# NikolausDemmel/rootba

Hardware: NVIDIA H100
Metric: ms/LM-iter (linearize+QR+PCG) on BAL at 1/2/4/8 H100 vs CPU ref (lower is better)
Workload: dtype f32

## Files before the change

rootba_b200/csrc/assembled.cuh:

```cuda
#pragma once

#include "kernels.cuh"

namespace rba {

struct AsmTerm {
  long long base;
  int ij, meta;
};

template <class S>
__global__ void __launch_bounds__(256) k_rcs_terms(const S* __restrict__ panel, const AsmTerm* __restrict__ terms, long long w0,
                                                   long long w1, int damping, S* __restrict__ stage) {
  using V2 = typename ST<S>::V2;
  const int lane = threadIdx.x & 31;
  const int g = lane / 9, p = lane - 9 * g;
  if (lane >= 27) return;
  const long long warps = (long long)gridDim.x * (blockDim.x >> 5);
  for (long long w = w0 + 3 * (blockIdx.x * (long long)(blockDim.x >> 5) + (threadIdx.x >> 5)) + g; w < w1; w += 3 * warps) {
    const AsmTerm at = terms[w];
    const int n = at.meta & 0x7fff, lg = (at.meta >> 15) & 7, KP = at.meta >> 18, G = 1 << lg;
    const int ia = at.ij & 0xffff, ib = at.ij >> 16;
    const int ca = 9 * ia + p, pa = ca >> 1;
    const int off_a = 2 * ((pa >> lg) * 32 + (pa & (G - 1))) + (ca & 1);
    const int cb0 = 9 * ib, pb0 = cb0 >> 1;
    const bool odd = cb0 & 1;
    int off_b[5];
#pragma unroll
    for (int k = 0; k < 5; ++k) off_b[k] = ((pb0 + k) >> lg) * 32 + ((pb0 + k) & (G - 1));
    const size_t rstride = (size_t)KP * 64;
    const S* __restrict__ lmp = panel + at.base;
    const int r0 = damping ? 2 * n - 3 : 0, r1 = damping ? 2 * n : 2 * n - 3;
    S acc[9];
#pragma unroll
    for (int q = 0; q < 9; ++q) acc[q] = 0;
#pragma unroll 3
    for (int r = r0; r < r1; ++r) {
      const S* row = lmp + (size_t)r * rstride;
      const V2* row2 = reinterpret_cast<const V2*>(row);
      const S va = __ldg(row + off_a);
      V2 b[5];
#pragma unroll
      for (int k = 0; k < 5; ++k) b[k] = __ldg(row2 + off_b[k]);
      const S el[10] = {b[0].x, b[0].y, b[1].x, b[1].y, b[2].x, b[2].y, b[3].x, b[3].y, b[4].x, b[4].y};
#pragma unroll
      for (int q = 0; q < 9; ++q) acc[q] = fma(va, odd ? el[q + 1] : el[q], acc[q]);
    }
    S* o = stage + 81 * (size_t)(w - w0) + 9 * p;
#pragma unroll
    for (int q = 0; q < 9; ++q) o[q] = acc[q];
  }
}

template <class S>
__global__ void k_rcs_combine(const int* __restrict__ blk_ptr, const int* __restrict__ wpos, int nblk, long long w0, long long w1,
                              const S* __restrict__ stage, const S* __restrict__ base, const int2* __restrict__ pos, int first,
                              S* __restrict__ out) {
  const long long i = blockIdx.x * (long long)blockDim.x + threadIdx.x;
  if (i >= 81LL * nblk) return;
  const int bi = (int)(i / 81), e = (int)(i - 81LL * bi);
  auto lower = [&](long long w) {
    int lo = blk_ptr[bi], hi = blk_ptr[bi + 1];
    while (lo < hi) {
      const int mid = (lo + hi) >> 1;
      if (wpos[mid] < w) lo = mid + 1; else hi = mid;
    }
    return lo;
  };
  const int t0 = lower(w0), t1 = lower(w1);
  const int2 ps = pos ? pos[bi] : make_int2(bi, -1);
  S* lo = out + 81 * (size_t)ps.x + e;
  if (t0 == t1 && !first) return;
  S s = first ? (base ? base[81 * (size_t)bi + e] : S(0)) : *lo;
  for (int t = t0; t < t1; ++t) s += stage[81 * (size_t)(wpos[t] - w0) + e];
  *lo = s;
  if (ps.y >= 0) out[81 * (size_t)ps.y + 9 * (e % 9) + e / 9] = s;
}

constexpr int SPMV_WARPS = 4;
constexpr int SPMV_UNROLL = 4;
template <class S>
__global__ void __launch_bounds__(SPMV_WARPS * 32) k_rcs_spmv(const int* __restrict__ row_ptr, const int* __restrict__ col,
                                                               const S* __restrict__ val, const S* __restrict__ x, S* __restrict__ y,
                                                               const int* done, int pdl) {
  __shared__ S part[SPMV_WARPS][81];
  if (done && *reinterpret_cast<const volatile int*>(done)) return;
  const int row = blockIdx.x, w = threadIdx.x >> 5, lane = threadIdx.x & 31;
  const int k0 = row_ptr[row], k1 = row_ptr[row + 1];
  int qe[3];
#pragma unroll
  for (int u = 0; u < 3; ++u) qe[u] = (lane + 32 * u) % 9;
  if (pdl) asm volatile("griddepcontrol.wait;" ::: "memory");
  if (done && *done) return;
  if (pdl) asm volatile("griddepcontrol.launch_dependents;" ::: "memory");
  S acc[3] = {0, 0, 0};
  for (int k = k0 + w; k < k1; k += SPMV_WARPS * SPMV_UNROLL) {
    S v[SPMV_UNROLL][3], xv[SPMV_UNROLL][3];
#pragma unroll
    for (int j = 0; j < SPMV_UNROLL; ++j) {
      const int kk = k + SPMV_WARPS * j;
      const bool in = kk < k1;
      const S* blk = val + 81 * (size_t)(in ? kk : k0);
      const S* xc = x + 9 * (size_t)(in ? __ldg(col + kk) : 0);
#pragma unroll
      for (int u = 0; u < 3; ++u) {
        const bool e_in = in && lane + 32 * u < 81;
        v[j][u] = e_in ? __ldg(blk + lane + 32 * u) : S(0);
        xv[j][u] = e_in ? __ldcg(xc + qe[u]) : S(0);
      }
    }
#pragma unroll
    for (int j = 0; j < SPMV_UNROLL; ++j)
#pragma unroll
      for (int u = 0; u < 3; ++u) acc[u] = fma(v[j][u], xv[j][u], acc[u]);
  }
#pragma unroll
  for (int u = 0; u < 3; ++u)
    if (lane + 32 * u < 81) part[w][lane + 32 * u] = acc[u];
  __syncthreads();
  if (threadIdx.x < 9) {
    const int p = threadIdx.x;
    S s = 0;
#pragma unroll
    for (int ww = 0; ww < SPMV_WARPS; ++ww)
#pragma unroll
      for (int q = 0; q < 9; ++q) s += part[ww][9 * p + q];
    y[9 * (size_t)row + p] = s;
  }
}

}
```

rootba_b200/csrc/solver.cu:

```cuda
#include <cuda_runtime.h>
#include <dlfcn.h>

#include <cstdio>
#include <cstdlib>
#include <cstring>
#include <chrono>
#include <limits>
#include <memory>
#include <string>
#include <vector>

#include "../../include/rootba_b200.h"
#include "../host/bal_io_fast.hpp"
#include "kernels.cuh"
#include "covariance.cuh"
#include "assembled.cuh"
#include "nccl_dyn.hpp"

namespace rba {

thread_local std::string g_err;

#define CU(call)                                                                                   \
  do {                                                                                             \
// ... 20 lines not shown
  virtual int set_state(const void* cams, const void* lms) = 0;
  virtual int get_state(void* cams, void* lms) = 0;
  virtual int backup() = 0;
  virtual int restore() = 0;
  virtual int set_camera_fixed(const uint8_t* flags) = 0;
  virtual int set_camera_prior(const void* mean, const void* sqrt_info) = 0;
  virtual int set_camera_pair_prior(int32_t num_pairs, const int32_t* pairs, const void* mean, const void* sqrt_info) = 0;
  virtual int set_landmark_prior(int32_t num, const int32_t* lm_idx, const void* mean, const void* sqrt_info) = 0;
  virtual int compute_error(rba_residual_info* out) = 0;
  virtual int linearize() = 0;
  virtual int solve(double lambda, void* inc_out, rba_cg_summary* cg) = 0;
  virtual int apply(const void* inc, void* l_diff_out, bool update_cameras) = 0;
  virtual int lm_step(bool linearize_first, double lambda, rba_lm_step_result* out) = 0;
  virtual int lm_run(const rba_lm_opts* o, int max_steps, rba_lm_iteration* log, int* steps_done, int* terminated, rba_stage_timings* totals) = 0;
  virtual int get_timings(rba_stage_timings* out) const = 0;
  virtual int get_stats(rba_workload_stats* out) const = 0;
  virtual int get_scaling(void* scaling, void* diag2) = 0;
  virtual int get_rhs(void* b) = 0;
  virtual int get_precond(void* inv, void* blocks) = 0;
  virtual int right_multiply(const void* x, void* y) = 0;
  virtual int debug_get_block(int lm, void* out, int rows, int cols, void* jls) = 0;
  virtual int compute_covariance(double* cam_cov, double* lm_cov) = 0;
  virtual int time_matvec(int reps, double* sec) = 0;
  virtual int timer_start() = 0;
  virtual int timer_stop(double* sec) = 0;
  virtual void* stream_ptr() = 0;
  virtual int synchronize() = 0;
  virtual int comm_init(const void* uid) = 0;
  virtual int ipc_export(void* out128) = 0;
  virtual int ipc_import(const void* all) = 0;
};

namespace rba {

template <class S>
struct Solver : rba_handle {
  static constexpr int EBLOCKS = 592;
  static constexpr int KPMAX = sizeof(S) == 4 ? 16 : 10;
  static constexpr int TILE_WARPS = 4;
  static constexpr int K1_CAP = 3904;
  static constexpr int K2_CAP = 3072;
  static constexpr int K4_WARPS = 4;
  static constexpr int K4_NS = 2;
  static constexpr int K4_STAGE = 4608;
  static constexpr size_t K4_SMEM_TMA = (size_t)K4_WARPS * K4_NS * K4_STAGE;
  static constexpr long long K4_ITEM_COST = 48;
  static constexpr int IMP_WARPS = 2, IMP_MAXSLOTS = 64, IMP_NS = 1;

  rba_solver_opts opt{};
  KOpts ko{};
  Layout L;
  int nc = 0, nl_total = 0;
  int device = 0;
  int sm_count = 132;
  cudaStream_t stream = nullptr;
  std::vector<void*> allocs;
  size_t device_bytes = 0;
  DevPtrs<S> D{};
  S* cams_bk = nullptr; S* lms_bk = nullptr;
  long long state_version = 0;
  rba_residual_info error_cache{}; long long error_cache_version = -1, error_enqueue_version = -1; bool error_cache_valid = false;
  bool error_enqueued = false;
  int* d_csr_obs_slots = nullptr; ReduceItem* d_csr_obs_items = nullptr; int* d_csr_obs_item_ptr = nullptr;
  int* d_csr_y_slots = nullptr; ReduceItem* d_csr_y_items = nullptr; int* d_csr_y_item_ptr = nullptr;
  int n_obs_items = 0, n_y_items = 0;
  const int* op_slots = nullptr; const ReduceItem* op_items = nullptr; const int* op_item_ptr = nullptr; int n_op_items = 0;
  bool implicit_op = false;
  bool panel_form = true;
  ReduceItem* d_pb_items = nullptr; int* d_pb_item_ptr = nullptr; int n_pb_items = 0;
  Scratch<S> k1_sc{}, k2_sc{};
  size_t k1_smem = 0, k2_smem = 0;
  int k1_max_blocks = 264, k2_max_blocks = 264;
  TileOrder order_k1{nullptr, 0}, order_kp{nullptr, 0};
  MatvecItem* d_items = nullptr;
  int n_dealt = 0, tma_grid = 1;
  size_t k4_smem_small = 0;
  int imp_tile_split = 0;
  size_t imp_smem = 0; int imp_grid = 1;
  int pcg_cluster = 16;
  bool pcg_partials = true;
  bool peer_ar = true;
  bool asm_hook = true;
  int asm_at = 0;
  int* h_prog = nullptr; int* d_prog = nullptr;
  int pcg_solve_id = 0;
  double* d_epart = nullptr;
  double* d_red = nullptr;
  int* d_flags = nullptr;
  int* d_cam_cnt = nullptr;
  PcgState* d_state = nullptr;
  PcgState* h_state = nullptr;
  struct PinnedResults {
    double error[6];
    int error_flags[4];
    int linearize_flags[4];
    double l_diff;
    int apply_flags[4];
  };
  PinnedResults* h_res = nullptr;
  cudaEvent_t poll_ev[2] = {nullptr, nullptr};
  bool linearized = false;
  bool new_linearization_point = false;
  bool have_inc = false;
  S last_lambda = 0;
  bool damping_valid = false;
  uint8_t* d_cam_fixed = nullptr;
  bool all_cams_fixed = false;
  bool has_abs_prior = false;
  S* d_prior_mean = nullptr;
  S* d_prior_L = nullptr;
  S* d_prior_A = nullptr;
  S* d_prior_r = nullptr;
  S* d_prior_H = nullptr;
  S* d_prior_g = nullptr;
  int n_pairs = 0, pair_cap = 0;
  int* d_pair_ij = nullptr;
  S* d_pair_mean = nullptr;
  S* d_pair_L = nullptr;
  S* d_pair_A = nullptr;
  S* d_pair_r = nullptr;
  int* d_pair_item = nullptr;
  int* d_pair_nbr = nullptr;
  S* d_pair_O = nullptr;
  int* d_pair_ptr = nullptr;
  S* d_pair_ov = nullptr;
  int n_lmp = 0, lmp_cap = 0;
  int* d_lmp_slot = nullptr;
  int* d_lmp_of_lm = nullptr;
  int* d_lmp_lm = nullptr;
  S* d_lmp_mean = nullptr;
  S* d_lmp_L = nullptr;
  S* d_lmp_Lg = nullptr;
  rba_stage_timings tm{};
  EventPair ev_stage1, ev_stage2, ev_precond, ev_pcg, ev_backsub, ev_update, ev_error, ev_mv, ev_user;
  long long launches = 0;
  long long lin_l0 = 0, solve_l0 = 0, apply_l0 = 0;
  NcclApi* nccl = nullptr;
  ncclComm_t comm = nullptr;
  char* peer_mem = nullptr;
  size_t peer_bytes = 0;
  PeerComm pc{};
  bool peer_ok = false;
  int ar_seq = 0, c_seq = 0, s_seq = 0;
  std::vector<void*> ipc_opened;
  bool cov_ready = false;
  int cov_nblk = 0;
  int2* d_cov_blk_cam = nullptr; int* d_cov_blk_ptr = nullptr; int2* d_cov_terms = nullptr;
  int* d_cov_lm_slot0 = nullptr; int* d_cov_lm_n = nullptr;
  bool asm_on = false, su_valid = false, s_valid = false;
  int asm_nblk = 0, asm_switch = 0; long long asm_nnzb = 0;
  std::vector<long long> asm_ranges;
  AsmTerm* d_asm_terms = nullptr; int* d_asm_wpos = nullptr; int* d_asm_blk_ptr = nullptr; int2* d_asm_pos = nullptr;
  int* d_asm_row_ptr = nullptr; int* d_asm_col = nullptr;
  S* d_asm_stage = nullptr; S* d_asm_Su = nullptr; S* d_asm_S = nullptr;

  ~Solver() override {
    if (comm && nccl) nccl->CommDestroy(comm);
    for (void* p : ipc_opened) cudaIpcCloseMemHandle(p);
    for (void* p : allocs) cudaFree(p);
    if (h_prog) cudaFreeHost(h_prog);
    if (h_state) cudaFreeHost(h_state);
    if (h_res) cudaFreeHost(h_res);
    for (EventPair* e : {&ev_stage1, &ev_stage2, &ev_precond, &ev_pcg, &ev_backsub, &ev_update, &ev_error, &ev_mv, &ev_user}) {
      if (e->a) cudaEventDestroy(e->a);
      if (e->b) cudaEventDestroy(e->b);
    }
    for (auto& e : poll_ev) if (e) cudaEventDestroy(e);
    if (stream) cudaStreamDestroy(stream);
  }

  template <class T>
  int dalloc(T** p, size_t count, bool zero = true) {
    const size_t bytes = std::max<size_t>(count, 1) * sizeof(T);
    void* q = nullptr;
    CU(cudaMalloc(&q, bytes));
    allocs.push_back(q);
    device_bytes += bytes;
    if (zero) CU(cudaMemsetAsync(q, 0, bytes, stream));
    *p = (T*)q;
    return RBA_OK;
  }
  int dfree(void* q) {
    if (!q) return RBA_OK;
    allocs.erase(std::find(allocs.begin(), allocs.end(), q));
    CU(cudaFree(q));
    return RBA_OK;
  }
  template <class T>
  int upload(T** p, const std::vector<T>& v) {
    int rc = dalloc(p, v.size(), false);
    if (rc) return rc;
    if (!v.empty()) CU(cudaMemcpyAsync(*p, v.data(), v.size() * sizeof(T), cudaMemcpyHostToDevice, stream));
    return RBA_OK;
  }

  int start(EventPair& e) { e.used = true; CU(cudaEventRecord(e.a, stream)); return RBA_OK; }
  int stop(EventPair& e) { CU(cudaEventRecord(e.b, stream)); return RBA_OK; }
  static double elapsed(EventPair& e) {
    if (!e.used) return 0.0;
    float ms = 0;
    if (cudaEventElapsedTime(&ms, e.a, e.b) != cudaSuccess) return 0.0;
    return 1e-3 * ms;
  }

  int init(const rba_problem_view* pv, const rba_solver_opts* o) {
    TRY(validate_options(*o));
    int ndev = 0;
    if (cudaGetDeviceCount(&ndev) != cudaSuccess || ndev == 0) {
      g_err = "no CUDA device: rootba_b200 has no CPU fallback";
      return RBA_ERR_NO_DEVICE;
    }
    if (opt.device >= 0) CU(cudaSetDevice(opt.device));
    CU(cudaGetDevice(&device));
    cudaDeviceProp prop;
    CU(cudaGetDeviceProperties(&prop, device));
    sm_count = prop.multiProcessorCount;
    CU(cudaStreamCreateWithFlags(&stream, cudaStreamNonBlocking));
    for (EventPair* e : {&ev_stage1, &ev_stage2, &ev_precond, &ev_pcg, &ev_backsub, &ev_update, &ev_error, &ev_mv, &ev_user}) {
      CU(cudaEventCreate(&e->a));
      CU(cudaEventCreate(&e->b));
    }
    for (auto& e : poll_ev) CU(cudaEventCreateWithFlags(&e, cudaEventDisableTiming));
    read_test_hooks();
    TRY(upload_layout(pv));
    TRY(deal_work());
    TRY(alloc_buffers());
    TRY(setup_assembled());
    TRY(setup_kernels());
    CU(cudaStreamSynchronize(stream));
    return RBA_OK;
  }

  int validate_options(const rba_solver_opts& o) {
    opt = o;
    if (opt.nranks < 1 || opt.rank < 0 || opt.rank >= opt.nranks) { g_err = "bad rank/nranks"; return RBA_ERR_INVALID_ARGUMENT; }
    if (opt.operator_form != 0 && opt.operator_form != 1) { g_err = "operator_form must be 0 (dense) or 1 (implicit)"; return RBA_ERR_INVALID_ARGUMENT; }
    if (opt.solver_type < 0 || opt.solver_type > 2) { g_err = "solver_type must be 0 (SQUARE_ROOT), 1 (SCHUR_COMPLEMENT) or 2 (POWER_SCHUR_COMPLEMENT)"; return RBA_ERR_INVALID_ARGUMENT; }
    if (opt.solver_type == 2 && opt.nranks > 1) { g_err = "POWER_SCHUR_COMPLEMENT runs on one GPU (the power-series vector kernel has no peer exchange yet)"; return RBA_ERR_UNSUPPORTED; }
    if (opt.stage2_form != 0 && opt.stage2_form != 1) { g_err = "stage2_form must be 0 (Q2 panel, reference) or 1 (orthogonality identity)"; return RBA_ERR_INVALID_ARGUMENT; }
    if (opt.pcg_check_period <= 0) opt.pcg_check_period = 4;
    if (opt.residual_reset_period <= 0) opt.residual_reset_period = 10;
    if (opt.power_order <= 0) opt.power_order = 20;
    implicit_op = opt.operator_form == 1 || opt.solver_type != 0;
    panel_form = !implicit_op && opt.stage2_form == 0;
    ko.use_valid_projections_only = opt.use_valid_projections_only;
    ko.robust_norm = opt.robust_norm;
    ko.write_panel = implicit_op ? 0 : 1;
    ko.huber = opt.huber_parameter;
    ko.jacobi_eps = opt.jacobi_scaling_epsilon > 0 ? opt.jacobi_scaling_epsilon : (double)ST<S>::eps_sqrt();
    return RBA_OK;
  }

  void read_test_hooks() {
    if (const char* e = getenv("RBA_PCG_PARTIALS")) pcg_partials = atoi(e) != 0;
    if (const char* e = getenv("RBA_PCG_CLUSTER")) pcg_cluster = std::max(1, std::min(atoi(e), 16));
    if (const char* e = getenv("RBA_PEER_AR")) peer_ar = atoi(e) != 0;
    if (const char* e = getenv("RBA_ASSEMBLED_RCS")) asm_hook = atoi(e) != 0;
    if (const char* e = getenv("RBA_ASSEMBLED_AT")) asm_at = std::max(0, atoi(e));
  }

  int upload_layout(const rba_problem_view* pv) {
    nc = pv->num_cameras;
    nl_total = pv->num_landmarks;
    std::string msg = build_layout(nc, nl_total, pv->lm_obs_offset, pv->obs_cam_idx, opt.rank, opt.nranks, KPMAX, L);
    if (!msg.empty()) { g_err = msg; return RBA_ERR_INVALID_ARGUMENT; }
    std::vector<S> xy((size_t)2 * L.nslots, S(0));
    const S* src = (const S*)pv->obs_xy;
    for (int s = 0; s < L.nslots; ++s)
      if (L.slot_obs[s] >= 0) { xy[2 * (size_t)s] = src[2 * L.slot_obs[s]]; xy[2 * (size_t)s + 1] = src[2 * L.slot_obs[s] + 1]; }
    TileInfo* d_tiles; int* d_sorted; int* d_slot_cam; int* d_slot_lm; S* d_xy;
    TRY(upload(&d_tiles, L.tiles));
    TRY(upload(&d_sorted, L.sorted_lm));
    TRY(upload(&d_slot_cam, L.slot_cam));
    TRY(upload(&d_slot_lm, L.slot_lm));
    TRY(upload(&d_xy, xy));
    D.tiles = d_tiles; D.ntiles = (int)L.tiles.size(); D.sorted_lm = d_sorted;
    D.slot_cam = d_slot_cam; D.slot_lm = d_slot_lm; D.slot_xy = d_xy; D.nslots = L.nslots; D.nc = nc;
    TRY(upload(&d_csr_obs_slots, L.csr_obs.slots));
    TRY(upload(&d_csr_obs_items, L.csr_obs.items));
    TRY(upload(&d_csr_obs_item_ptr, L.csr_obs.cam_item_ptr));
    n_obs_items = (int)L.csr_obs.items.size();
    if (L.csr_y_is_obs) {
      d_csr_y_slots = d_csr_obs_slots; d_csr_y_items = d_csr_obs_items; d_csr_y_item_ptr = d_csr_obs_item_ptr;
      n_y_items = n_obs_items;
    } else {
      TRY(upload(&d_csr_y_slots, L.csr_y.slots));
      TRY(upload(&d_csr_y_items, L.csr_y.items));
      TRY(upload(&d_csr_y_item_ptr, L.csr_y.cam_item_ptr));
      n_y_items = (int)L.csr_y.items.size();
    }
    if (implicit_op) { op_slots = d_csr_obs_slots; op_items = d_csr_obs_items; op_item_ptr = d_csr_obs_item_ptr; n_op_items = n_obs_items; }
    else { op_slots = d_csr_y_slots; op_items = d_csr_y_items; op_item_ptr = d_csr_y_item_ptr; n_op_items = n_y_items; }
    TRY(upload(&d_pb_items, L.pb_items));
    TRY(upload(&d_pb_item_ptr, L.pb_cam_item_ptr));
    n_pb_items = (int)L.pb_items.size();
    return RBA_OK;
  }

  int deal_work() {
    if (implicit_op) {
      while (imp_tile_split < (int)L.tiles.size() && (32 / L.tiles[imp_tile_split].G) * L.tiles[imp_tile_split].n <= IMP_MAXSLOTS) ++imp_tile_split;
      imp_smem = (size_t)IMP_WARPS * IMP_NS * (size_t)IMP_MAXSLOTS * 48 * sizeof(S);
      CU(cudaFuncSetAttribute((k_matvec_implicit_tma<S, IMP_WARPS, IMP_MAXSLOTS, IMP_NS>), cudaFuncAttributeMaxDynamicSharedMemorySize, (int)imp_smem));
      int bps = 0;
      CU(cudaOccupancyMaxActiveBlocksPerMultiprocessor(&bps, (k_matvec_implicit_tma<S, IMP_WARPS, IMP_MAXSLOTS, IMP_NS>), IMP_WARPS * 32, imp_smem));
      imp_grid = std::max(1, std::min((imp_tile_split + IMP_WARPS - 1) / IMP_WARPS, sm_count * std::max(1, bps)));
// ... 968 lines not shown
      L2.terminated = terminated ? 1 : 0;
    }
    *steps_done = it;
    *terminated_out = terminated ? 1 : 0;
    return RBA_OK;
  }

  int get_timings(rba_stage_timings* out) const override { *out = tm; out->kernel_launches = launches; return RBA_OK; }
  int get_stats(rba_workload_stats* out) const override {
    std::memset(out, 0, sizeof(*out));
    out->num_landmarks_local = L.nl_local;
    out->num_observations_local = L.nobs_local;
    out->sum_n2 = L.sum_n2;
    out->max_n = L.max_n;
    out->num_tiles = (int)L.tiles.size();
    out->panel_scalars = L.panel_scalars;
    out->panel_scalars_algorithmic = 18 * L.sum_n2;
    out->device_bytes = (int64_t)device_bytes;
    out->matvec_algorithmic_bytes = s_valid ? (81 * asm_nnzb + 18 * (int64_t)nc) * (int64_t)sizeof(S) + 4 * (asm_nnzb + nc + 1)
                                           : (18 * L.sum_n2 + 18 * L.nobs_local) * (int64_t)sizeof(S) + 4 * L.nobs_local;
    out->landmark_begin = L.lm_begin;
    out->landmark_end = L.lm_end;
    out->num_matvec_items = (int)L.items.size();
    return RBA_OK;
  }

  int get_scaling(void* scaling, void* diag2) override {
    if (scaling) CU(cudaMemcpyAsync(scaling, D.scaling, (size_t)9 * nc * sizeof(S), cudaMemcpyDeviceToHost, stream));
    if (diag2) CU(cudaMemcpyAsync(diag2, D.diag2, (size_t)9 * nc * sizeof(S), cudaMemcpyDeviceToHost, stream));
    CU(cudaStreamSynchronize(stream));
    return RBA_OK;
  }
  int get_rhs(void* b) override {
    CU(cudaMemcpyAsync(b, D.b, (size_t)9 * nc * sizeof(S), cudaMemcpyDeviceToHost, stream));
    CU(cudaStreamSynchronize(stream));
    return RBA_OK;
  }
  int get_precond(void* inv, void* blocks) override {
    if (inv) CU(cudaMemcpyAsync(inv, D.inv, (size_t)81 * nc * sizeof(S), cudaMemcpyDeviceToHost, stream));
    if (blocks) CU(cudaMemcpyAsync(blocks, D.blocks, (size_t)81 * nc * sizeof(S), cudaMemcpyDeviceToHost, stream));
    CU(cudaStreamSynchronize(stream));
    return RBA_OK;
  }
  int right_multiply(const void* x, void* y) override {
    if (!linearized || !damping_valid) { g_err = "rba_right_multiply needs rba_linearize + rba_solve first"; return RBA_ERR_STATE; }
    CU(cudaMemcpyAsync(D.z, x, (size_t)9 * nc * sizeof(S), cudaMemcpyHostToDevice, stream));
    CU(cudaMemsetAsync(D.y, 0, (size_t)9 * nc * sizeof(S), stream));
    TRY(matvec_launch(D.z));
    TRY(allreduce(D.y, (size_t)9 * nc));
    k_pcg_q<S><<<NPART, 128, 0, stream>>>(D, D.y, D.z, D.y, last_lambda);
    ++launches;
    CU(cudaMemcpyAsync(y, D.y, (size_t)9 * nc * sizeof(S), cudaMemcpyDeviceToHost, stream));
    CU(cudaStreamSynchronize(stream));
    CU(cudaGetLastError());
    return RBA_OK;
  }

  int time_matvec(int reps, double* sec) override {
    if (!linearized || !damping_valid) { g_err = "rba_time_matvec needs rba_linearize + rba_solve first"; return RBA_ERR_STATE; }
    TRY(matvec_launch(D.p));
    TRY(start(ev_mv));
    for (int r = 0; r < reps; ++r) TRY(matvec_launch(D.p));
    TRY(stop(ev_mv));
    CU(cudaStreamSynchronize(stream));
    CU(cudaGetLastError());
    *sec = elapsed(ev_mv) / std::max(reps, 1);
    tm.matvec_time = *sec;
    return RBA_OK;
  }

  int timer_start() override { return start(ev_user); }
  int timer_stop(double* sec) override {
    int rc = stop(ev_user); if (rc) return rc;
    CU(cudaStreamSynchronize(stream));
    *sec = elapsed(ev_user);
    return RBA_OK;
  }
  void* stream_ptr() override { return (void*)stream; }
  int synchronize() override { CU(cudaStreamSynchronize(stream)); return RBA_OK; }

  struct PairTerms {
    std::vector<int> slot0, nn;
    std::vector<int2> blk_cam;
    std::vector<int> blk_ptr;
    std::vector<int2> terms;
    std::vector<int> wpos;
  };
  int pair_terms(PairTerms& P) {
    const int nl = L.nl_local;
    P.slot0.resize(nl); P.nn.resize(nl);
    long long nt = 0;
    for (int lm = 0; lm < nl; ++lm) {
      const int sidx = L.sorted_of_lm[lm];
      const TileInfo& T = L.tiles[L.tile_of_sorted[sidx]];
      P.slot0[lm] = T.slot_base + (sidx - T.lm_base) * T.n;
      P.nn[lm] = T.n;
      nt += (long long)T.n * (T.n + 1) / 2;
    }
    if (nt > std::numeric_limits<int>::max()) { g_err = "more than 2^31 camera-pair terms"; return RBA_ERR_UNSUPPORTED; }
    std::vector<int2> raw;
    raw.reserve((size_t)nt);
    for (int lm = 0; lm < nl; ++lm)
      for (int a = 0; a < P.nn[lm]; ++a)
        for (int b = 0; b <= a; ++b) raw.push_back(make_int2(P.slot0[lm] + a, P.slot0[lm] + b));
    std::vector<int> idx(raw.size()), tmp(raw.size());
    std::iota(idx.begin(), idx.end(), 0);
    std::vector<long long> cnt((size_t)nc + 1);
    auto pass = [&](const std::vector<int>& src, std::vector<int>& dst, bool by_a) {
      std::fill(cnt.begin(), cnt.end(), 0LL);
      for (int w : src) ++cnt[L.slot_cam[by_a ? raw[w].x : raw[w].y] + 1];
      for (int c = 0; c < nc; ++c) cnt[c + 1] += cnt[c];
      for (int w : src) dst[cnt[L.slot_cam[by_a ? raw[w].x : raw[w].y]]++] = w;
    };
    pass(idx, tmp, false);
    pass(tmp, idx, true);
    tmp.clear(); tmp.shrink_to_fit();
    P.terms.resize(raw.size());
    for (size_t t = 0; t < idx.size(); ++t) P.terms[t] = raw[idx[t]];
    P.wpos.swap(idx);
    P.blk_cam.clear(); P.blk_ptr.clear();
    for (size_t t = 0; t < P.terms.size(); ++t) {
      const int2 cc = make_int2(L.slot_cam[P.terms[t].x], L.slot_cam[P.terms[t].y]);
      if (t == 0 || cc.x != P.blk_cam.back().x || cc.y != P.blk_cam.back().y) {
        P.blk_cam.push_back(cc);
        P.blk_ptr.push_back((int)t);
      }
    }
    P.blk_ptr.push_back((int)P.terms.size());
    return RBA_OK;
  }

  int setup_assembled() {
    if (!asm_hook || opt.nranks != 1 || implicit_op) return RBA_OK;
    PairTerms P;
    TRY(pair_terms(P));
    const long long nblk = (long long)P.blk_cam.size(), nt = (long long)P.terms.size();
    long long ndiag = 0;
    for (const int2& c : P.blk_cam) ndiag += c.x == c.y;
    const long long nnzb = 2 * nblk - ndiag;
    const size_t s_bytes = (size_t)nnzb * 81 * sizeof(S);
    if (4 * s_bytes > (size_t)L.panel_scalars * sizeof(S)) return RBA_OK;
    const long long cap = std::max<long long>(1, ((long long)2 << 30) / (81 * (long long)sizeof(S)));
    std::vector<long long> ranges{0};
    long long w = 0, stage_terms = 0;
    for (int lm = 0; lm < L.nl_local; ++lm) {
      const long long k = (long long)P.nn[lm] * (P.nn[lm] + 1) / 2;
      if (w + k - ranges.back() > cap && w > ranges.back()) ranges.push_back(w);
      w += k;
      stage_terms = std::max(stage_terms, w - ranges.back());
    }
    ranges.push_back(nt);
    if (ranges.size() > 2) return RBA_OK;
    const size_t need = s_bytes + (size_t)(nblk + stage_terms) * 81 * sizeof(S) + (size_t)nt * (sizeof(AsmTerm) + sizeof(int)) +
                        (size_t)(nblk + nnzb + nc + 2) * sizeof(int) + (size_t)nblk * sizeof(int2);
    size_t free_b = 0, total_b = 0;
    CU(cudaMemGetInfo(&free_b, &total_b));
    if (need + ((size_t)256 << 20) > free_b) return RBA_OK;
    std::vector<int> row_ptr((size_t)nc + 1, 0), colv((size_t)nnzb);
    for (const int2& c : P.blk_cam) { ++row_ptr[c.x + 1]; if (c.x != c.y) ++row_ptr[c.y + 1]; }
    for (int c = 0; c < nc; ++c) row_ptr[c + 1] += row_ptr[c];
    std::vector<int> fill(row_ptr.begin(), row_ptr.end() - 1);
    std::vector<int2> posv((size_t)nblk);
    for (long long b = 0; b < nblk; ++b) {
      const int2 c = P.blk_cam[b];
      const int lo = fill[c.x]++;
      colv[lo] = c.y;
      int up = -1;
      if (c.x != c.y) { up = fill[c.y]++; colv[up] = c.x; }
      posv[b] = make_int2(lo, up);
    }
    std::vector<AsmTerm> at;
    at.reserve((size_t)nt);
    for (int lm = 0; lm < L.nl_local; ++lm) {
      const int sidx = L.sorted_of_lm[lm];
      const TileInfo& T = L.tiles[L.tile_of_sorted[sidx]];
      const int g = sidx - T.lm_base;
      for (int a = 0; a < T.n; ++a)
        for (int b = 0; b <= a; ++b)
          at.push_back({T.panel_off + 2LL * g * T.G, a | b << 16, T.n | (31 - __builtin_clz((unsigned)T.G)) << 15 | (int)T.KP << 18});
    }
    TRY(upload(&d_asm_terms, at));
    TRY(upload(&d_asm_wpos, P.wpos));
    TRY(upload(&d_asm_blk_ptr, P.blk_ptr));
    TRY(upload(&d_asm_pos, posv));
    TRY(upload(&d_asm_row_ptr, row_ptr));
    TRY(upload(&d_asm_col, colv));
    TRY(dalloc(&d_asm_stage, (size_t)stage_terms * 81, false));
    TRY(dalloc(&d_asm_Su, (size_t)nblk * 81));
    TRY(dalloc(&d_asm_S, (size_t)nnzb * 81));
    asm_ranges = ranges;
    asm_nblk = (int)nblk; asm_nnzb = nnzb;
    const double staged = 4.0 * (double)nt * 81 * sizeof(S), saved = (double)L.panel_scalars * sizeof(S) - (double)s_bytes;
    asm_switch = asm_at > 0 ? asm_at : 1 + (int)std::ceil(2.0 * staged / std::max(saved, 1.0));
    asm_on = true;
    return RBA_OK;
  }
  void assemble(int damping) {
    for (size_t k = 0; k + 1 < asm_ranges.size(); ++k) {
      const long long w0 = asm_ranges[k], w1 = asm_ranges[k + 1];
      const int grid = (int)std::max<long long>(1, std::min<long long>((w1 - w0 + 23) / 24, (long long)sm_count * 16));
      k_rcs_terms<S><<<grid, 256, 0, stream>>>(D.panel, d_asm_terms, w0, w1, damping, d_asm_stage);
      k_rcs_combine<S><<<(unsigned)((81LL * asm_nblk + 255) / 256), 256, 0, stream>>>(
          d_asm_blk_ptr, d_asm_wpos, asm_nblk, w0, w1, d_asm_stage, damping ? (const S*)d_asm_Su : nullptr,
          damping ? (const int2*)d_asm_pos : nullptr, (int)(k == 0), damping ? d_asm_S : d_asm_Su);
      launches += 2;
    }
  }

  template <class T>
  int cov_upload(T** p, const std::vector<T>& v) {
    void* q = nullptr;
    CU(cudaMalloc(&q, std::max<size_t>(v.size(), 1) * sizeof(T)));
    allocs.push_back(q);
    if (!v.empty()) CU(cudaMemcpy(q, v.data(), v.size() * sizeof(T), cudaMemcpyHostToDevice));
    *p = (T*)q;
    return RBA_OK;
  }
  int cov_build_lists() {
    if (cov_ready) return RBA_OK;
    PairTerms P;
    TRY(pair_terms(P));
    TRY(cov_upload(&d_cov_blk_cam, P.blk_cam));
    TRY(cov_upload(&d_cov_blk_ptr, P.blk_ptr));
    TRY(cov_upload(&d_cov_terms, P.terms));
    TRY(cov_upload(&d_cov_lm_slot0, P.slot0));
    TRY(cov_upload(&d_cov_lm_n, P.nn));
    cov_nblk = (int)P.blk_cam.size();
    cov_ready = true;
    return RBA_OK;
  }
  template <bool TA, bool TB>
  void cov_gemm(long long M, long long N, long long K, double alpha, const double* A, long long lda, const double* B, long long ldb,
                double beta, double* C, long long ldc, int lower, int ktri) {
    k_cov_dgemm<TA, TB><<<dim3((unsigned)(M / COV_TB), (unsigned)(N / COV_TB)), 256, 0, stream>>>((int)M, (int)N, (int)K, alpha, A, lda, B,
                                                                                                   ldb, beta, C, ldc, lower, ktri);
  }
  int cov_copy(double* dst, long long dld, const double* src, long long sld, long long rows, long long cols) {
    CU(cudaMemcpy2DAsync(dst, dld * sizeof(double), src, sld * sizeof(double), rows * sizeof(double), cols, cudaMemcpyDeviceToDevice, stream));
    return RBA_OK;
  }
  int compute_covariance(double* cam_cov, double* lm_cov) override {
    if (!cam_cov && !lm_cov) { g_err = "rba_compute_covariance: cam_cov and lm_cov are both NULL"; return RBA_ERR_INVALID_ARGUMENT; }
    if (opt.nranks > 1) {
      g_err = "rba_compute_covariance: sharded handles (nranks > 1) are not supported: the reduced camera matrix would need a cross-rank sum";
      return RBA_ERR_UNSUPPORTED;
    }
    TRY(cov_build_lists());
    constexpr long long TB = COV_TB;
    const long long n = 9LL * nc, np = (n + TB - 1) / TB * TB, ns = L.nslots;
    const int nl = L.nl_local, nt = (int)(np / TB);
    size_t total = 0;
    auto carve = [&](size_t bytes) { const size_t o = total; total += (bytes + 255) & ~size_t(255); return o; };
    const size_t o_A = carve((size_t)(np * np) * 8), o_W = carve((size_t)(np * TB) * 8), o_Y = carve((size_t)(np * TB) * 8),
                 o_T = carve((size_t)(TB * TB) * 8), o_d = carve((size_t)np * 8), o_jp = carve((size_t)ns * 18 * 8),
                 o_kb = carve((size_t)ns * 27 * 8), o_wl = carve((size_t)nl * 9 * 8), o_rk = carve((size_t)nl * 4), o_fail = carve(4),
                 o_cam = carve((size_t)nc * 81 * 8), o_lm = carve(lm_cov ? (size_t)nl * 9 * 8 : 0);
    size_t free_b = 0, total_b = 0;
    CU(cudaMemGetInfo(&free_b, &total_b));
    if (total > free_b) {
      g_err = "rba_compute_covariance needs " + std::to_string(total) + " bytes of device memory (a dense " + std::to_string(n) + " x " +
              std::to_string(n) + " float64 reduced camera matrix plus scratch); " + std::to_string(free_b) + " bytes are free";
      return RBA_ERR_UNSUPPORTED;
    }
    char* base = nullptr;
    CU(cudaMalloc(&base, total));
    struct CovScratch { char* p; ~CovScratch() { cudaFree(p); } } scratch{base};
    double* A = (double*)(base + o_A); double* W = (double*)(base + o_W); double* Y = (double*)(base + o_Y);
    double* Tt = (double*)(base + o_T); double* d = (double*)(base + o_d); double* jp = (double*)(base + o_jp);
    double* kb = (double*)(base + o_kb); double* wl = (double*)(base + o_wl); int* rk = (int*)(base + o_rk);
    int* fail = (int*)(base + o_fail); double* cam_out = (double*)(base + o_cam); double* lm_out = (double*)(base + o_lm);
    CU(cudaMemsetAsync(A, 0, (size_t)(np * np) * 8, stream));
    CU(cudaMemsetAsync(fail, 0x7f, 4, stream));
    const int wgrid = std::max(1, std::min((nl + 3) / 4, sm_count * 16));
    if (n_lmp > 0)
      k_cov_landmark<S, true><<<wgrid, 128, 0, stream>>>(D, ko, d_cov_lm_slot0, d_cov_lm_n, nl, jp, kb, wl, rk, d_lmp_of_lm);
    else
      k_cov_landmark<S><<<wgrid, 128, 0, stream>>>(D, ko, d_cov_lm_slot0, d_cov_lm_n, nl, jp, kb, wl, rk);
    k_cov_assemble<<<std::max(1, std::min((cov_nblk + 7) / 8, sm_count * 8)), 256, 0, stream>>>(d_cov_blk_cam, d_cov_blk_ptr, d_cov_terms,
                                                                                                  cov_nblk, jp, kb, A, np);
    if (has_abs_prior || n_pairs > 0)
      k_cov_priors<S><<<(nc + 127) / 128, 128, 0, stream>>>(D.cams, nc, has_abs_prior ? d_prior_mean : nullptr, d_prior_L, d_pair_ij,
                                                            d_pair_mean, d_pair_L, n_pairs > 0 ? d_pair_ptr : nullptr, d_pair_item,
                                                            d_pair_nbr, A, np);
    k_cov_diag<<<(unsigned)((np + 255) / 256), 256, 0, stream>>>(A, np, n, np, D.cam_fixed, d);
    k_cov_equil<<<dim3((unsigned)(np / 32), (unsigned)(np / 8)), dim3(32, 8), 0, stream>>>(A, np, n, np, D.cam_fixed, d);
    for (int k = 0; k < nt; ++k) {
      const long long k0 = k * TB, m = np - k0 - TB;
      k_cov_tile_potrf<<<1, 256, 0, stream>>>(A, np, k0, COV_PIVOT_TAU, fail);
      if (m == 0) break;
      k_cov_tile_trtri<<<1, COV_TB, 0, stream>>>(A, np, k0, Tt, TB);
      double* P = A + (k0 + TB) + k0 * np;
      TRY(cov_copy(W, m, P, np, m, TB));
      cov_gemm<false, true>(m, TB, TB, 1.0, W, m, Tt, TB, 0.0, P, np, 0, 0);
      cov_gemm<false, true>(m, m, TB, -1.0, P, np, P, np, 1.0, P + TB * np, np, 1, 0);
    }
    int h_fail = 0;
    CU(cudaMemcpyAsync(&h_fail, fail, sizeof(int), cudaMemcpyDeviceToHost, stream));
    CU(cudaStreamSynchronize(stream));
    CU(cudaGetLastError());
    if (h_fail < n) {
      static const char* names[9] = {"tx", "ty", "tz", "rx", "ry", "rz", "f", "k1", "k2"};
      g_err = "rba_compute_covariance: the reduced camera matrix is singular: Cholesky pivot <= " + std::to_string(COV_PIVOT_TAU) +
              " of the equilibrated matrix at camera " + std::to_string(h_fail / 9) + ", increment entry " + std::to_string(h_fail % 9) +
              " (" + names[h_fail % 9] + "). The gauge is not fixed, or a free camera has no observation and no prior: hold parameters "
              "with rba_set_camera_fixed or add priors with rba_set_camera_prior";
      return RBA_NUMERICAL_FAILURE;
    }
    for (int j = nt - 1; j >= 0; --j) {
      const long long j0 = j * TB, m = np - j0 - TB;
      k_cov_tile_trtri<<<1, COV_TB, 0, stream>>>(A, np, j0, Tt, TB);
      if (m > 0) {
        double* P = A + (j0 + TB) + j0 * np;
        TRY(cov_copy(W, m, P, np, m, TB));
        cov_gemm<false, false>(m, TB, m, 1.0, P + TB * np, np, W, m, 0.0, Y, m, 0, 1);
        cov_gemm<false, false>(m, TB, TB, -1.0, Y, m, Tt, TB, 0.0, P, np, 0, 0);
      }
      TRY(cov_copy(A + j0 + j0 * np, np, Tt, TB, TB, TB));
    }
    for (int i = 0; i < nt; ++i) {
      const long long r0 = i * TB, kk = np - r0 - TB;
      if (r0 > 0) {
        TRY(cov_copy(W, TB, A + r0, np, TB, r0));
        cov_gemm<true, false>(TB, r0, TB, 1.0, A + r0 + r0 * np, np, W, TB, 0.0, A + r0, np, 0, 0);
      }
      k_cov_tile_lauu2<<<1, 256, 0, stream>>>(A, np, r0);
      if (kk > 0) cov_gemm<true, false>(TB, r0 + TB, kk, 1.0, A + (r0 + TB) + r0 * np, np, A + (r0 + TB), np, 1.0, A + r0, np, 0, 0);
    }
    if (cam_cov) {
      k_cov_cam_out<<<(81 * nc + 255) / 256, 256, 0, stream>>>(A, np, d, D.cam_fixed, nc, cam_out);
      CU(cudaMemcpyAsync(cam_cov, cam_out, (size_t)81 * nc * sizeof(double), cudaMemcpyDeviceToHost, stream));
    }
    if (lm_cov) {
      k_cov_lm_marginal<<<wgrid, 128, 0, stream>>>(A, np, d, D.cam_fixed, D.slot_cam, d_cov_lm_slot0, d_cov_lm_n, nl, kb, wl, rk, lm_out);
      CU(cudaMemcpyAsync(lm_cov, lm_out, (size_t)9 * nl * sizeof(double), cudaMemcpyDeviceToHost, stream));
    }
    CU(cudaGetLastError());
    CU(cudaStreamSynchronize(stream));
    return RBA_OK;
  }

  int debug_get_block(int lm, void* out, int rows, int cols, void* jls_out) override {
    if (lm < L.lm_begin || lm >= L.lm_end) { g_err = "landmark not in this shard"; return RBA_ERR_INVALID_ARGUMENT; }
    const int sidx = L.sorted_of_lm[lm - L.lm_begin];
    const TileInfo& T = L.tiles[L.tile_of_sorted[sidx]];
    const int n = T.n, G = T.G, KP = T.KP, g = sidx - T.lm_base;
    const int pad = (4 - (9 * n) % 4) % 4, lm_idx = 9 * n + pad, res_idx = lm_idx + 3;
    if (rows != 2 * n + 3 || cols != res_idx + 1) { g_err = "block dims mismatch"; return RBA_ERR_INVALID_ARGUMENT; }
    if (!D.panel) { g_err = "rba_debug_get_block needs operator_form = 0 (no Q2 panels are stored for the implicit operator)"; return RBA_ERR_UNSUPPORTED; }
    CU(cudaStreamSynchronize(stream));
    std::vector<S> panel((size_t)2 * n * KP * 64), rec((size_t)28 * n), lmk(24);
    const int slot0 = T.slot_base + g * n;
    CU(cudaMemcpy(panel.data(), D.panel + T.panel_off, panel.size() * sizeof(S), cudaMemcpyDeviceToHost));
    CU(cudaMemcpy(rec.data(), D.q1d + (size_t)28 * slot0, rec.size() * sizeof(S), cudaMemcpyDeviceToHost));
    CU(cudaMemcpy(lmk.data(), D.lmk + (size_t)24 * sidx, 24 * sizeof(S), cudaMemcpyDeviceToHost));
// ... 277 lines not shown
```

Before: 6.252.

## Stage term outputs through shared memory and add direct damping assembly kernel

k_rcs_terms now writes each warp's three 9x9 term blocks into shared memory and then copies them to the global stage buffer contiguously, so the global stores coalesce instead of each lane writing nine strided values. When a damping buffer (D.dmp) exists, the damped Schur assembly skips the panel-based term pass and the combine pass. A new k_rcs_damping kernel instead adds the damping-row outer products directly from the compact dmp array onto Su. This needs an extra pair_terms upload and assumes the dmp layout of 28-strided 3x9 rows matches the panel's damping rows.

```diff
diff --git a/rootba_b200/csrc/assembled.cuh b/rootba_b200/csrc/assembled.cuh
--- a/rootba_b200/csrc/assembled.cuh
+++ b/rootba_b200/csrc/assembled.cuh
@@ -9,46 +9,55 @@
   int ij, meta;
 };
 
+constexpr int RCS_TERMS_WARPS = 8;
 template <class S>
-__global__ void __launch_bounds__(256) k_rcs_terms(const S* __restrict__ panel, const AsmTerm* __restrict__ terms, long long w0,
-                                                   long long w1, int damping, S* __restrict__ stage) {
+__global__ void __launch_bounds__(RCS_TERMS_WARPS * 32) k_rcs_terms(const S* __restrict__ panel, const AsmTerm* __restrict__ terms,
+                                                                    long long w0, long long w1, int damping, S* __restrict__ stage) {
   using V2 = typename ST<S>::V2;
-  const int lane = threadIdx.x & 31;
+  __shared__ S buf[RCS_TERMS_WARPS][243];
+  const int lane = threadIdx.x & 31, wib = threadIdx.x >> 5;
   const int g = lane / 9, p = lane - 9 * g;
-  if (lane >= 27) return;
-  const long long warps = (long long)gridDim.x * (blockDim.x >> 5);
-  for (long long w = w0 + 3 * (blockIdx.x * (long long)(blockDim.x >> 5) + (threadIdx.x >> 5)) + g; w < w1; w += 3 * warps) {
-    const AsmTerm at = terms[w];
-    const int n = at.meta & 0x7fff, lg = (at.meta >> 15) & 7, KP = at.meta >> 18, G = 1 << lg;
-    const int ia = at.ij & 0xffff, ib = at.ij >> 16;
-    const int ca = 9 * ia + p, pa = ca >> 1;
-    const int off_a = 2 * ((pa >> lg) * 32 + (pa & (G - 1))) + (ca & 1);
-    const int cb0 = 9 * ib, pb0 = cb0 >> 1;
-    const bool odd = cb0 & 1;
-    int off_b[5];
+  const long long warps = (long long)gridDim.x * RCS_TERMS_WARPS;
+  for (long long w3 = w0 + 3 * (blockIdx.x * (long long)RCS_TERMS_WARPS + wib); w3 < w1; w3 += 3 * warps) {
+    const long long w = w3 + g;
+    if (lane < 27 && w < w1) {
+      const AsmTerm at = terms[w];
+      const int n = at.meta & 0x7fff, lg = (at.meta >> 15) & 7, KP = at.meta >> 18, G = 1 << lg;
+      const int ia = at.ij & 0xffff, ib = at.ij >> 16;
+      const int ca = 9 * ia + p, pa = ca >> 1;
+      const int off_a = 2 * ((pa >> lg) * 32 + (pa & (G - 1))) + (ca & 1);
+      const int cb0 = 9 * ib, pb0 = cb0 >> 1;
+      const bool odd = cb0 & 1;
+      int off_b[5];
 #pragma unroll
-    for (int k = 0; k < 5; ++k) off_b[k] = ((pb0 + k) >> lg) * 32 + ((pb0 + k) & (G - 1));
-    const size_t rstride = (size_t)KP * 64;
-    const S* __restrict__ lmp = panel + at.base;
-    const int r0 = damping ? 2 * n - 3 : 0, r1 = damping ? 2 * n : 2 * n - 3;
-    S acc[9];
+      for (int k = 0; k < 5; ++k) off_b[k] = ((pb0 + k) >> lg) * 32 + ((pb0 + k) & (G - 1));
+      const size_t rstride = (size_t)KP * 64;
+      const S* __restrict__ lmp = panel + at.base;
+      const int r0 = damping ? 2 * n - 3 : 0, r1 = damping ? 2 * n : 2 * n - 3;
+      S acc[9];
 #pragma unroll
-    for (int q = 0; q < 9; ++q) acc[q] = 0;
+      for (int q = 0; q < 9; ++q) acc[q] = 0;
 #pragma unroll 3
-    for (int r = r0; r < r1; ++r) {
-      const S* row = lmp + (size_t)r * rstride;
-      const V2* row2 = reinterpret_cast<const V2*>(row);
-      const S va = __ldg(row + off_a);
-      V2 b[5];
+      for (int r = r0; r < r1; ++r) {
+        const S* row = lmp + (size_t)r * rstride;
+        const V2* row2 = reinterpret_cast<const V2*>(row);
+        const S va = __ldg(row + off_a);
+        V2 b[5];
 #pragma unroll
-      for (int k = 0; k < 5; ++k) b[k] = __ldg(row2 + off_b[k]);
-      const S el[10] = {b[0].x, b[0].y, b[1].x, b[1].y, b[2].x, b[2].y, b[3].x, b[3].y, b[4].x, b[4].y};
+        for (int k = 0; k < 5; ++k) b[k] = __ldg(row2 + off_b[k]);
+        const S el[10] = {b[0].x, b[0].y, b[1].x, b[1].y, b[2].x, b[2].y, b[3].x, b[3].y, b[4].x, b[4].y};
 #pragma unroll
-      for (int q = 0; q < 9; ++q) acc[q] = fma(va, odd ? el[q + 1] : el[q], acc[q]);
+        for (int q = 0; q < 9; ++q) acc[q] = fma(va, odd ? el[q + 1] : el[q], acc[q]);
+      }
+      S* o = buf[wib] + 9 * lane;
+#pragma unroll
+      for (int q = 0; q < 9; ++q) o[q] = acc[q];
     }
-    S* o = stage + 81 * (size_t)(w - w0) + 9 * p;
-#pragma unroll
-    for (int q = 0; q < 9; ++q) o[q] = acc[q];
+    __syncwarp();
+    const int cnt = 81 * (int)min(3LL, w1 - w3);
+    S* dst = stage + 81 * (size_t)(w3 - w0);
+    for (int i = lane; i < cnt; i += 32) dst[i] = buf[wib][i];
+    __syncwarp();
   }
 }
 
@@ -75,6 +84,27 @@
   for (int t = t0; t < t1; ++t) s += stage[81 * (size_t)(wpos[t] - w0) + e];
   *lo = s;
   if (ps.y >= 0) out[81 * (size_t)ps.y + 9 * (e % 9) + e / 9] = s;
+}
+
+template <class S>
+__global__ void k_rcs_damping(const int* __restrict__ blk_ptr, const int2* __restrict__ pair_terms, int nblk, const S* __restrict__ dmp,
+                              const S* __restrict__ Su, const int2* __restrict__ pos, S* __restrict__ out) {
+  const long long i = blockIdx.x * (long long)blockDim.x + threadIdx.x;
+  if (i >= 81LL * nblk) return;
+  const int bi = (int)(i / 81), e = (int)(i - 81LL * bi), p = e / 9, q = e - 9 * p;
+  S s = Su[i];
+  for (int t = blk_ptr[bi]; t < blk_ptr[bi + 1]; ++t) {
+    const int2 st = __ldg(pair_terms + t);
+    const S* da = dmp + 28 * (size_t)st.x + p;
+    const S* db = dmp + 28 * (size_t)st.y + q;
+    S v = fma(__ldg(da), __ldg(db), S(0));
+    v = fma(__ldg(da + 9), __ldg(db + 9), v);
+    v = fma(__ldg(da + 18), __ldg(db + 18), v);
+    s += v;
+  }
+  const int2 ps = pos[bi];
+  out[81 * (size_t)ps.x + e] = s;
+  if (ps.y >= 0) out[81 * (size_t)ps.y + 9 * q + p] = s;
 }
 
 constexpr int SPMV_WARPS = 4;
diff --git a/rootba_b200/csrc/solver.cu b/rootba_b200/csrc/solver.cu
--- a/rootba_b200/csrc/solver.cu
+++ b/rootba_b200/csrc/solver.cu
@@ -196,6 +196,7 @@
   std::vector<long long> asm_ranges;
   AsmTerm* d_asm_terms = nullptr; int* d_asm_wpos = nullptr; int* d_asm_blk_ptr = nullptr; int2* d_asm_pos = nullptr;
   int* d_asm_row_ptr = nullptr; int* d_asm_col = nullptr;
+  int2* d_asm_pair_terms = nullptr;
   S* d_asm_stage = nullptr; S* d_asm_Su = nullptr; S* d_asm_S = nullptr;
 
   ~Solver() override {
@@ -1470,7 +1471,7 @@
     ranges.push_back(nt);
     if (ranges.size() > 2) return RBA_OK;
     const size_t need = s_bytes + (size_t)(nblk + stage_terms) * 81 * sizeof(S) + (size_t)nt * (sizeof(AsmTerm) + sizeof(int)) +
-                        (size_t)(nblk + nnzb + nc + 2) * sizeof(int) + (size_t)nblk * sizeof(int2);
+                        (size_t)(nblk + nnzb + nc + 2) * sizeof(int) + (size_t)nblk * sizeof(int2) + (D.dmp ? (size_t)nt * sizeof(int2) : 0);
     size_t free_b = 0, total_b = 0;
     CU(cudaMemGetInfo(&free_b, &total_b));
     if (need + ((size_t)256 << 20) > free_b) return RBA_OK;
@@ -1503,6 +1504,7 @@
     TRY(upload(&d_asm_pos, posv));
     TRY(upload(&d_asm_row_ptr, row_ptr));
     TRY(upload(&d_asm_col, colv));
+    if (D.dmp) TRY(upload(&d_asm_pair_terms, P.terms));
     TRY(dalloc(&d_asm_stage, (size_t)stage_terms * 81, false));
     TRY(dalloc(&d_asm_Su, (size_t)nblk * 81));
     TRY(dalloc(&d_asm_S, (size_t)nnzb * 81));
@@ -1514,10 +1516,16 @@
     return RBA_OK;
   }
   void assemble(int damping) {
+    if (damping && D.dmp) {
+      k_rcs_damping<S><<<(unsigned)((81LL * asm_nblk + 255) / 256), 256, 0, stream>>>(d_asm_blk_ptr, d_asm_pair_terms, asm_nblk, D.dmp,
+                                                                                    d_asm_Su, d_asm_pos, d_asm_S);
+      ++launches;
+      return;
+    }
     for (size_t k = 0; k + 1 < asm_ranges.size(); ++k) {
       const long long w0 = asm_ranges[k], w1 = asm_ranges[k + 1];
       const int grid = (int)std::max<long long>(1, std::min<long long>((w1 - w0 + 23) / 24, (long long)sm_count * 16));
-      k_rcs_terms<S><<<grid, 256, 0, stream>>>(D.panel, d_asm_terms, w0, w1, damping, d_asm_stage);
+      k_rcs_terms<S><<<grid, RCS_TERMS_WARPS * 32, 0, stream>>>(D.panel, d_asm_terms, w0, w1, damping, d_asm_stage);
       k_rcs_combine<S><<<(unsigned)((81LL * asm_nblk + 255) / 256), 256, 0, stream>>>(
           d_asm_blk_ptr, d_asm_wpos, asm_nblk, w0, w1, d_asm_stage, damping ? (const S*)d_asm_Su : nullptr,
           damping ? (const int2*)d_asm_pos : nullptr, (int)(k == 0), damping ? d_asm_S : d_asm_Su);
```

After: 6.000, median of 6. 1.04x faster.
